# yxtay/transformer-recommenders

Measured on AMD Instinct MI355X. Metric: user-sequences/sec (train step) MovieLens-1M seq200 d128 @1/2/4/8 GPU, higher is better.
Workload: dtype bf16; 1 GPU; MovieLens-1M-shaped: 3883 items, seq_len=200, d_model=128, 4-layer causal BERT (heads=4, ffn=512), InfoNCELoss over in-batch shared negatives, AdamW; per_gpu_batch=512, global_batch=512, seq_len=200, lengths=dense, loss_heads_evaluated=all 7 + LogitsStatistics (reference training_step), parallelism=dp1, launch=eager launches

## Files before the change

### transformer-recommenders_amd/csrc/encoder.hip

```cpp
#include <math.h>
#include <stdlib.h>
#include <new>
#include <string.h>

#include "internal.h"

namespace {

struct LayerParams {
  int64_t wqkv, bqkv, wo, bo, ln1g, ln1b, w1, b1, w2, b2, ln2g, ln2b;
};
struct ParamLayout {
  int64_t pos, type, eg, eb;
  int64_t total;
};

int64_t layer_base(const xfmr_encoder_cfg* c, int i, ParamLayout* pl) {
  const int64_t H = c->hidden, I = c->inter;
  pl->pos = 0;
  pl->type = pl->pos + (int64_t)c->max_pos * H;
  pl->eg = pl->type + 2 * H;
  pl->eb = pl->eg + H;
  const int64_t first = pl->eb + H;
  const int64_t per = 3 * H * H + 3 * H + H * H + H + 2 * H + I * H + I + H * I + H + 2 * H;
// ... 48 lines not shown
  const int64_t i = (int64_t)blockIdx.x * 256 + threadIdx.x;
  if (i < n4) xf_st4<true>(dst, 4 * i, *reinterpret_cast<const float4*>(src + 4 * i));
}

bool mixed_storage(const xfmr_encoder_cfg* c) {
  static const bool force_fp32 = [] {
    const char* e = getenv("XFMR_ACT_FP32");
    return e && *e && *e != '0';
  }();
  return c->precision == XFMR_PREC_BF16 && !force_fp32;
}
int prof(const xfmr_encoder_cfg* c, int kind, int layer, int which, hipStream_t st) {
  if (c->profile_kernel != kind || c->profile_layer != layer || !c->profile_events[which]) return XFMR_OK;
  return hipEventRecord((hipEvent_t)c->profile_events[which], st) == hipSuccess ? XFMR_OK : XFMR_EHIP;
}
bool ln_fused(const xfmr_encoder_cfg* c, int64_t T) {
  static const int64_t min_tokens = [] { const char* e = getenv("XFMR_LN_FUSED_MIN_TOKENS"); return e ? (int64_t)atoll(e) : (int64_t)12288; }();
  return mixed_storage(c) && c->hidden == 128 && T >= min_tokens && !(c->flags & XFMR_ENC_LN_UNFUSED);
}
bool ln_store_x() {
  const char* e = getenv("XFMR_LN_STORE_X");
  return e && *e && *e != '0';
}
bool ffn_fused(const xfmr_encoder_cfg* c, int64_t T) {
  return ln_fused(c, T) && T >= 16384 && (c->inter % 128) == 0 && c->inter <= 1024 && !(c->flags & XFMR_ENC_FFN_UNFUSED);
}

constexpr int64_t kDwSideTokens = 40960;
bool dw_side_shape(const xfmr_encoder_cfg* c, int64_t T) {
  if (!mixed_storage(c) || c->layers > 64) return false;
  return (c->flags & XFMR_ENC_DW_SIDE_ANY) || (c->hidden == 128 && T >= kDwSideTokens);
}

Acts carve(const xfmr_encoder_cfg* c, unsigned char* base, int layer, LayerActs* la, RedBufs* rb = nullptr) {
  const size_t T = (size_t)c->batch * c->seq_len, H = c->hidden, I = c->inter, A = c->heads;
  const size_t es = mixed_storage(c) ? 2 : 4;
  size_t o = 0;
  auto take_bytes = [&](size_t bytes) -> void* {
    void* p = base ? base + o : nullptr;
    o += up256(bytes);
// ... 185 lines not shown
  if (acts_bytes < a.total) return XFMR_EWORKSPACE;
  const int B = cfg->batch, L = cfg->seq_len, H = cfg->hidden, I = cfg->inter, A = cfg->heads;
  const int64_t Tplan = (int64_t)B * L;
  const int32_t* const offs = cfg->seq_offsets;
  const int64_t T = offs ? cfg->packed_rows : Tplan;
  const int prec = cfg->precision;
  const bool mix = mixed_storage(cfg);
  const bool causal = !(cfg->flags & XFMR_ENC_BIDIRECTIONAL);
  hipStream_t st = (hipStream_t)stream;
  const XfSeed sd(cfg->seed, cfg->step_device);
  ParamLayout pl;
  layer_base(cfg, 0, &pl);
  const bool fuse_ln = ln_fused(cfg, Tplan);
  const bool fuse_ffn = ffn_fused(cfg, Tplan);
  const bool rederive = fuse_ln && !ln_store_x();
  float* const x0 = rederive ? nullptr : a.x0;
  if (offs) {
    XF_TRY(xf_embed_ln_fwd_packed_ex(item_idx, table, n_rows, params + pl.pos, params + pl.type, params + pl.eg,
                                     params + pl.eb, x0, mix ? a.x0b : nullptr, a.emb_pre, a.emb_mean, a.emb_rstd, key_mask,
                                     T, cfg->row_pos, H, cfg->ln_eps, cfg->hidden_dropout, sd, SITE_EMB, st));
  } else {
    XF_TRY(xf_embed_ln_fwd_ex(item_idx, table, n_rows, params + pl.pos, params + pl.type, params + pl.eg,
                              params + pl.eb, x0, mix ? a.x0b : nullptr, a.emb_pre, a.emb_mean, a.emb_rstd, key_mask, B,
                              L, H, cfg->ln_eps, cfg->hidden_dropout, sd, SITE_EMB, st));
  }
  if (cfg->embed_event && hipEventRecord((hipEvent_t)cfg->embed_event, st) != hipSuccess) return XFMR_EHIP;
  const float* x = x0;
  XfLnResidual xr{a.emb_pre, a.emb_mean, a.emb_rstd, params + pl.eg, params + pl.eb, cfg->hidden_dropout, SITE_EMB};
  const void* xg = mix ? a.x0b : (const void*)a.x0;
  const uint32_t sA = mix ? XF_S16_A : 0;
// ... 294 lines not shown
```

### transformer-recommenders_amd/csrc/gemm.hip

```cpp
#include <stdio.h>
#include <stdlib.h>

#include <algorithm>
#include <type_traits>

#include "internal.h"

#define XF_PIN_SCALAR(x) asm volatile("" : "+v"(x))
#ifndef XF_LN_DIAG
#define XF_LN_DIAG 0
#endif
#ifndef XF_GEMM_PF
#define XF_GEMM_PF 1
#endif
#ifndef XF_DW_PF
#define XF_DW_PF 1
#endif
#ifdef XF_FFN_STAMP
#define XF_STAMP(i) do { if (stamp_on) st_buf[(i)] = __builtin_readcyclecounter(); } while (0)
#else
#define XF_STAMP(i) do {} while (0)
#endif
#ifndef XF_FFN_ASM_BARRIER
#define XF_FFN_ASM_BARRIER 1
// ... 20 lines not shown

namespace {

enum { EPI_STORE = 0, EPI_GELU = 1, EPI_DROP_RES = 2, EPI_GELU_GRAD = 3, EPI_SPLITK = 4, EPI_DROP_RES_LN = 5,
       EPI_DX_LNBWD = 6, EPI_DROP_RES_LN_RE = 7, EPI_DROP_RES_LN_RED = 8 };
constexpr bool epi_res_ln(int epi) { return epi == EPI_DROP_RES_LN || epi == EPI_DROP_RES_LN_RE || epi == EPI_DROP_RES_LN_RED; }
constexpr int epi_res_mode(int epi) { return epi == EPI_DROP_RES_LN_RE ? 1 : epi == EPI_DROP_RES_LN_RED ? 2 : 0; }

struct GemmArgs {
  const void* A; const void* B; void* C;
  int64_t lda, ldb, ldc;
  int64_t M; int N; int K;
  int k_chunk;
  int nt_n, nt_m, nt_z;
  int nt_full, short_rows;
  const float* bias;
  const float* R;
  const void* P;
  void* C2;
  int aux_grad;
  uint32_t s16;
  float* bias_part;
  XfDropout drop;
  const float* ln_gamma; const float* ln_beta; float ln_eps;
  float* Y; void* Y16; float* ln_mean; float* ln_rstd;
  const float* rp_pre; const float* rp_mean; const float* rp_rstd; const float* rp_gamma; const float* rp_beta;
  XfDropout rp_drop;
  const float* lnb_x; const float* lnb_mean; const float* lnb_rstd;
  void* D16; float* lnb_partials;
  XfDropout drop2;
// ... 201 lines not shown
  return n;
}
static void xf_plan_row_tiles(GemmArgs& g, int BM) {
  g.nt_full = 0; g.short_rows = 0;
  g.nt_m = (int)((g.M + BM - 1) / BM);
  static const bool on = [] { const char* e = getenv("XFMR_ROW_TILES_SHORT"); return e && *e && *e != '0'; }();
  const int64_t cus = xf_num_cus();
  const int64_t per_cu = g.M / (BM * cus), rem = g.M - per_cu * BM * cus;
  if (!on || per_cu < 1 || rem <= 0 || rem > 32 * cus) return;
  const int64_t each = (((rem + cus - 1) / cus) + 15) / 16 * 16;
  g.nt_full = (int)(per_cu * cus);
  g.short_rows = (int)each;
  g.nt_m = g.nt_full + (int)((rem + each - 1) / each);
}

template <int RES>
__device__ __forceinline__ void epi_drop_res_ln_64x128(const f32x16 (&acc)[2], unsigned char* smem, const GemmArgs& g,
                                                       const int64_t m0, const int wid, const int lane) {
  constexpr int LPRL = 16, RPPL = 4, NPL = 4, WM = 32, WN = 64, NI = 2, SCR_LD = WN + 4;
  constexpr int64_t LDC = 128;
  const int wr = wid >> 1, wc = wid & 1;
  float* const scr = reinterpret_cast<float*>(smem) + wid * (16 * SCR_LD);
  float* const red = reinterpret_cast<float*>(smem) + 4 * 16 * SCR_LD;
  const int prow = lane / LPRL, li = lane % LPRL, c0 = li * 4;
  const int n = wc * WN + c0;
  const float4 bias = g.bias ? *reinterpret_cast<const float4*>(g.bias + n) : make_float4(0, 0, 0, 0);
  float4 gp = make_float4(0, 0, 0, 0), bp = gp;
  if constexpr (RES != 0) {
    gp = *reinterpret_cast<const float4*>(g.rp_gamma + n);
    bp = *reinterpret_cast<const float4*>(g.rp_beta + n);
  }
  float4 vv[2][NPL];
#pragma unroll
  for (int hf = 0; hf < 2; ++hf) {
    const int64_t mb = m0 + wr * WM + 16 * hf;
    float4 aux[NPL];
    float amu[NPL], ars[NPL];
#pragma unroll
    for (int ps = 0; ps < NPL; ++ps) {
      aux[ps] = make_float4(0, 0, 0, 0);
      amu[ps] = ars[ps] = 0.f;
      const int64_t m = mb + prow + RPPL * ps;
      if constexpr (RES == 0) {
        if (m < g.M) aux[ps] = *reinterpret_cast<const float4*>(g.R + m * LDC + n);
      } else if (m < g.M) {
        aux[ps] = *reinterpret_cast<const float4*>(g.rp_pre + m * LDC + n);
        amu[ps] = g.rp_mean[m];
        ars[ps] = g.rp_rstd[m];
      }
    }
#pragma unroll
    for (int j = 0; j < NI; ++j)
#pragma unroll
      for (int r = 0; r < 8; ++r)
        scr[(xf_acc_row(8 * hf + r, lane) - 16 * hf) * SCR_LD + j * 32 + (lane & 31)] = acc[j][8 * hf + r];
    __builtin_amdgcn_s_waitcnt(0xc07f);
    __builtin_amdgcn_wave_barrier();
#pragma unroll
    for (int ps = 0; ps < NPL; ++ps) {
      const int row = prow + RPPL * ps;
      const int64_t m = mb + row;
      float4 v = *reinterpret_cast<const float4*>(scr + row * SCR_LD + c0);
      v.x += bias.x; v.y += bias.y; v.z += bias.z; v.w += bias.w;
      if (g.drop.on) {
        xf_drop4(g.drop, (uint32_t)m, (uint32_t)(n), v);
      }
      float4 res = aux[ps];
      if constexpr (RES != 0) {
        XF_PIN_SCALAR(amu[ps]);
        XF_PIN_SCALAR(ars[ps]);
        res = xf_ln_out_drop4<RES == 2>(res, amu[ps], ars[ps], gp, bp, g.rp_drop, (uint32_t)m, (uint32_t)(n));
      }
      v.x += res.x; v.y += res.y; v.z += res.z; v.w += res.w;
      if (m >= g.M) v = make_float4(0, 0, 0, 0);
      else *reinterpret_cast<float4*>(reinterpret_cast<float*>(g.C) + m * LDC + n) = v;
      vv[hf][ps] = v;
    }
    __builtin_amdgcn_s_waitcnt(0xc07f);
    __builtin_amdgcn_wave_barrier();
  }
  XF_EPI_BARRIER();
  auto row_reduce = [&](float x) { return xf_row16_sum(x); };
  float mean[2][NPL];
#pragma unroll
  for (int hf = 0; hf < 2; ++hf)
#pragma unroll
    for (int ps = 0; ps < NPL; ++ps) {
      const float4 v = vv[hf][ps];
      const float s = row_reduce((v.x + v.y) + (v.z + v.w));
      if (li == 0) red[(wr * 2 + wc) * 32 + 16 * hf + prow + RPPL * ps] = s;
    }
  XF_EPI_BARRIER();
#pragma unroll
  for (int hf = 0; hf < 2; ++hf)
#pragma unroll
    for (int ps = 0; ps < NPL; ++ps) {
      const int rr = 16 * hf + prow + RPPL * ps;
      mean[hf][ps] = (red[(wr * 2) * 32 + rr] + red[(wr * 2 + 1) * 32 + rr]) * (1.f / 128.f);
    }
  XF_EPI_BARRIER();
#pragma unroll
  for (int hf = 0; hf < 2; ++hf)
#pragma unroll
    for (int ps = 0; ps < NPL; ++ps) {
      float4& v = vv[hf][ps];
      const float mu = mean[hf][ps];
      v.x -= mu; v.y -= mu; v.z -= mu; v.w -= mu;
      const float s = row_reduce((v.x * v.x + v.y * v.y) + (v.z * v.z + v.w * v.w));
      if (li == 0) red[(wr * 2 + wc) * 32 + 16 * hf + prow + RPPL * ps] = s;
    }
  XF_EPI_BARRIER();
  const float4 gm = *reinterpret_cast<const float4*>(g.ln_gamma + n);
  const float4 bt = *reinterpret_cast<const float4*>(g.ln_beta + n);
#pragma unroll
  for (int hf = 0; hf < 2; ++hf)
#pragma unroll
    for (int ps = 0; ps < NPL; ++ps) {
      const int rr = 16 * hf + prow + RPPL * ps;
      const int64_t m = m0 + wr * WM + rr;
      const float var = (red[(wr * 2) * 32 + rr] + red[(wr * 2 + 1) * 32 + rr]) * (1.f / 128.f);
      const float rs = rsqrtf(var + g.ln_eps);
      if (m >= g.M) continue;
      const float4 o = xf_ln_affine4(vv[hf][ps], rs, gm, bt);
      if (g.Y) *reinterpret_cast<float4*>(g.Y + m * LDC + n) = o;
      if (g.Y16) xf_st4<true>(g.Y16, m * LDC + n, o);
      if (wc == 0 && li == 0) {
        g.ln_mean[m] = mean[hf][ps];
        g.ln_rstd[m] = rs;
      }
    }
}

__device__ __forceinline__ void epi_dx_lnbwd_64x128(const f32x16 (&acc)[2], unsigned char* smem, const GemmArgs& g,
// ... 94 lines not shown
#pragma unroll
    for (int o = LPRL; o < 64; o <<= 1) {
      v.x += __shfl_xor(v.x, o, 64); v.y += __shfl_xor(v.y, o, 64);
      v.z += __shfl_xor(v.z, o, 64); v.w += __shfl_xor(v.w, o, 64);
    }
  };
  fold(dgam); fold(dbet); fold(dbias);
  if (prow == 0) {
    *reinterpret_cast<float4*>(&colred[(wr * 3 + 0) * 128 + n]) = dgam;
    *reinterpret_cast<float4*>(&colred[(wr * 3 + 1) * 128 + n]) = dbet;
    *reinterpret_cast<float4*>(&colred[(wr * 3 + 2) * 128 + n]) = dbias;
  }
  XF_EPI_BARRIER();
  for (int o = threadIdx.x; o < 3 * 128; o += 256)
    g.lnb_partials[(int64_t)tile_m * 3 * 128 + o] = colred[o] + colred[3 * 128 + o];
}

template <class P, int BM, int BN, int BK, bool TA, bool TB, int EPI, uint32_t S>
__device__ __forceinline__ void gemm_body(const GemmArgs& g_in, const int bid) {
  GemmArgs g = g_in;
  if (EPI != EPI_SPLITK) XF_CHAIN_PRIO();
  g.drop = xf_drop_resolve(g.drop); g.drop2 = xf_drop_resolve(g.drop2);
  if constexpr (EPI == EPI_DROP_RES_LN_RED) g.rp_drop = xf_drop_resolve(g.rp_drop);
  using elem = typename P::elem;
  using TileA = OperandTile<P, BM, BK, TA>;
  using TileB = OperandTile<P, BN, BK, TB>;
  using FA = Frag<P, TA>;
  using FB = Frag<P, TB>;
  constexpr bool a16 = S & XF_S16_A, b16 = S & XF_S16_B, c16 = S & XF_S16_C, p16 = S & XF_S16_P;
  static_assert(S == 0 || sizeof(elem) == 2, "bf16 storage needs the bf16 policy");
// ... 2 lines not shown
  constexpr size_t SCR_BYTES = (size_t)4 * 16 * SCR_LD * sizeof(float);
  constexpr size_t RED_BYTES = epi_res_ln(EPI) ? (size_t)4 * 32 * sizeof(float)
                               : EPI == EPI_DX_LNBWD  ? (size_t)(2 * 2 * 2 * 16 * 2 + 2 * 3 * 128) * sizeof(float)
                                                      : 0;
  constexpr size_t EPI_BYTES = SCR_BYTES + RED_BYTES;
  __shared__ __attribute__((aligned(16))) unsigned char smem[OPER_BYTES > EPI_BYTES ? OPER_BYTES : EPI_BYTES];
  elem* const sA = reinterpret_cast<elem*>(smem);
  elem* const sB = sA + TileA::IMG_ELEMS;

  const int lane = threadIdx.x & 63, wid = threadIdx.x >> 6;
  const int wr = wid >> 1, wc = wid & 1;
  constexpr int WM = BM / 2, WN = BN / 2, MI = WM / 32, NI = WN / 32;
  const TileIdx tix = tile_of(g.nt_n, g.nt_m, g.nt_z, bid);
  if (!tix.valid) return;
  const int64_t m0 = (epi_res_ln(EPI) || EPI == EPI_DX_LNBWD) ? xf_tile_rows(g, tix.m, BM) : (int64_t)tix.m * BM;
  const int n0 = tix.n * BN;
  int kbeg = 0, kend = g.K;
  if (g.k_chunk > 0) {
    kbeg = tix.z * g.k_chunk;
    kend = min(g.K, kbeg + g.k_chunk);
  }

  f32x16 acc[MI][NI];
#pragma unroll
  for (int i = 0; i < MI; ++i)
#pragma unroll
    for (int j = 0; j < NI; ++j)
#pragma unroll
      for (int r = 0; r < 16; ++r) acc[i][j][r] = 0.f;

// ... 231 lines not shown
    xf_static_for<NW>([&](auto ic) {
      constexpr int i = decltype(ic)::value;
      const int p = tid + i * 256, row = p / PC, ch = p % PC;
      reg[i] = *reinterpret_cast<const bf16x8*>(W2 + (int64_t)row * I + c * CH + ch * 8);
    });
  }
  __device__ __forceinline__ void commit_w2(__bf16* sW, int tid) const {
    xf_static_for<NW>([&](auto ic) {
      constexpr int i = decltype(ic)::value;
      const int p = tid + i * 256, row = p / PC, ch = p % PC;
      *reinterpret_cast<bf16x8*>(sW + row * LDC + ch * 8) = reg[i];
    });
  }
};

template <int CH, bool RE = false>
__global__ __launch_bounds__(256, CH == 128 ? XF_FFN_MIN_WAVES : 3) void ffn_fwd_fused_kernel(const FfnFwdArgs f_in) {
  FfnFwdArgs f = f_in;
  XF_CHAIN_PRIO();
  f.e.drop = xf_drop_resolve(f.e.drop);
  constexpr int H = 128, LDH = H + 8, LDC = CH + 8, BM = 64;
  constexpr int NJ = CH / 64;
  constexpr int W_ELEMS = CH * LDH > H * LDC ? CH * LDH : H * LDC;
  __shared__ __attribute__((aligned(16))) __bf16 sG[BM * LDC];
  __shared__ __attribute__((aligned(16))) __bf16 sW[W_ELEMS];
  __shared__ float sB1[1024];
  static_assert(W_ELEMS >= BM * LDH, "the x tile is staged through sW");
  static_assert(W_ELEMS * 2 >= 4 * 16 * 68 * 4 + 128 * 4, "the LayerNorm epilogue's scratch aliases sW");
  using FR = Frag<PrecBF16, false>;
  const int lane = threadIdx.x & 63, wid = threadIdx.x >> 6, tid = threadIdx.x;
  const int wr = wid >> 1, wc = wid & 1;
  const TileIdx tix = tile_of(1, f.e.nt_m, 1);
  if (!tix.valid) return;
  const int64_t m0 = xf_tile_rows(f.e, tix.m, BM);
  const int64_t M = f.e.M;
  const int I = f.I, nchunk = I / CH;
#ifdef XF_FFN_STAMP
  const bool stamp_on = f.stamps && threadIdx.x == 0;
  unsigned long long* st_buf = f.stamps + (int64_t)blockIdx.x * 64;
#endif
  XF_STAMP(0);

  WeightChunk<CH> wa, wb;
  constexpr int PC = CH / 8;

  {
    uint4 xr[4];
#pragma unroll
    for (int i = 0; i < 4; ++i) {
      const int p = tid + i * 256, row = p >> 4, ch = p & 15;
      xr[i] = make_uint4(0u, 0u, 0u, 0u);
      if (m0 + row < M) xr[i] = *reinterpret_cast<const uint4*>(f.X + (m0 + row) * H + ch * 8);
    }
    wa.load_w1(f.W1, 0, tid);
    wb.load_w2(f.W2, I, 0, tid);
    for (int i = tid; i < I; i += 256) sB1[i] = f.b1[i];
#pragma unroll
    for (int i = 0; i < 4; ++i) {
      const int p = tid + i * 256, row = p >> 4, ch = p & 15;
      *reinterpret_cast<uint4*>(sW + row * LDH + ch * 8) = xr[i];
    }
  }
  __syncthreads();
  bf16x8 xa[H / 16];
#pragma unroll
  for (int ks = 0; ks < H / 16; ++ks) xa[ks] = FR::get(sW, LDH, wr * 32, ks * 16);
  XF_STAMP(1);

  f32x16 accy[2];
#pragma unroll
  for (int j = 0; j < 2; ++j)
#pragma unroll
    for (int r = 0; r < 16; ++r) accy[j][r] = 0.f;

  for (int c = 0; c < nchunk; ++c) {
    XF_LOOP_BARRIER();
    if (c < 2) XF_STAMP(2 + 6 * c);
    wa.commit_w1(sW, tid);
    XF_LOOP_BARRIER();
    if (c < 2) XF_STAMP(3 + 6 * c);
    if (c + 1 < nchunk) wa.load_w1(f.W1, c + 1, tid);
    f32x16 accu[NJ];
#pragma unroll
    for (int j = 0; j < NJ; ++j)
#pragma unroll
      for (int r = 0; r < 16; ++r) accu[j][r] = 0.f;
    {
      bf16x8 fb[2][NJ];
#pragma unroll
      for (int j = 0; j < NJ; ++j) fb[0][j] = FR::get(sW, LDH, wc * (CH / 2) + j * 32, 0);
#pragma unroll
      for (int ks = 0; ks < H / 16; ++ks) {
        if (ks + 1 < H / 16) {
#pragma unroll
          for (int j = 0; j < NJ; ++j) fb[(ks + 1) & 1][j] = FR::get(sW, LDH, wc * (CH / 2) + j * 32, (ks + 1) * 16);
        }
#pragma unroll
        for (int j = 0; j < NJ; ++j) accu[j] = xf_mma(xa[ks], fb[ks & 1][j], accu[j]);
      }
    }
#pragma unroll
    for (int j = 0; j < NJ; ++j) {
      const int col = wc * (CH / 2) + j * 32 + (lane & 31);
      const float b = sB1[c * CH + col];
#pragma unroll
      for (int r = 0; r < 16; ++r) sG[(wr * 32 + xf_acc_row(r, lane)) * LDC + col] = (__bf16)(accu[j][r] + b);
    }
    if (c < 2) XF_STAMP(4 + 6 * c);
    XF_LOOP_BARRIER();
    if (c < 2) XF_STAMP(5 + 6 * c);
#pragma unroll
    for (int i = 0; i < BM * PC / 256; ++i) {
      const int p = tid + i * 256, row = p / PC, ch = p % PC;
      float4* cell = reinterpret_cast<float4*>(sG + row * LDC + ch * 8);
      const float4 u8 = *cell;
      const float4 g8 = xf_gelu_bf16x8(u8);
      if (m0 + row < M) {
        if (f.U) *reinterpret_cast<float4*>(f.U + (m0 + row) * I + c * CH + ch * 8) = u8;
        if (f.G) *reinterpret_cast<float4*>(f.G + (m0 + row) * I + c * CH + ch * 8) = g8;
      }
      *cell = g8;
    }
    wb.commit_w2(sW, tid);
    if (c < 2) XF_STAMP(6 + 6 * c);
    XF_LOOP_BARRIER();
    if (c < 2) XF_STAMP(7 + 6 * c);
    if (c + 1 < nchunk) wb.load_w2(f.W2, I, c + 1, tid);
#pragma unroll
    for (int ks = 0; ks < CH / 16; ++ks) {
      const bf16x8 fa = FR::get(sG, LDC, wr * 32, ks * 16);
      bf16x8 fb[2];
#pragma unroll
      for (int j = 0; j < 2; ++j) fb[j] = FR::get(sW, LDC, wc * 64 + j * 32, ks * 16);
#pragma unroll
      for (int j = 0; j < 2; ++j) accy[j] = xf_mma(fa, fb[j], accy[j]);
    }
  }
  XF_STAMP(14);
  __syncthreads();
  XF_STAMP(15);
  epi_drop_res_ln_64x128<RE ? 1 : 0>(accy, reinterpret_cast<unsigned char*>(sW), f.e, m0, wid, lane);
  XF_STAMP(16);
}

struct FfnBwdArgs {
  const __bf16* DY;
  const __bf16* W2;
  const __bf16* U;
  const __bf16* W1;
  __bf16* DI;
  int I;
  GemmArgs e;
};

__global__ __launch_bounds__(256, 3) void ffn_bwd_dx_fused_kernel(const FfnBwdArgs f_in) {
  FfnBwdArgs f = f_in;
  XF_CHAIN_PRIO();
// ... 278 lines not shown
    static const TileOverride dw = [] {
      TileOverride o{0, 0, 0};
      if (const char* e = getenv("XFMR_DW_TILE")) sscanf(e, "%d,%d", &o.bm, &o.bn);
      return o;
    }();
    if (dw.bm) { bm = dw.bm; bn = dw.bn; }
  }
  const TileOverride ov = tile_override();
  if (ov.bm && !epi_res_ln(EPI) && EPI != EPI_DX_LNBWD) { bm = ov.bm; bn = ov.bn; }
  dim3 block(256);
  static const int pad_lds = [] { const char* e = getenv("XFMR_GEMM_PAD_LDS"); return e ? atoi(e) : 0; }();
  GemmArgs ga = g;
  ga.nt_n = (int)((g.N + bn - 1) / bn);
  ga.nt_m = (int)((g.M + bm - 1) / bm);
  if (epi_res_ln(EPI) || EPI == EPI_DX_LNBWD) xf_plan_row_tiles(ga, bm);
  ga.nt_z = splits;
  const int64_t groups = splits > 1 ? (splits + 7) / 8 : (ga.nt_m + 7) / 8;
  const int64_t per = splits > 1 ? (int64_t)ga.nt_n * ga.nt_m : ga.nt_n;
  if (groups * per * 8 > 0x7fffffffll) return XFMR_EUNSUPPORTED;
  dim3 grid((unsigned)(groups * per * 8));
  if (bm == 64 && bn == 128) hipLaunchKernelGGL((gemm_kernel<P, 64, 128, BK, TA, TB, EPI, S>), grid, block, pad_lds, st, ga);
  else if (bm == 128 && bn == 64) hipLaunchKernelGGL((gemm_kernel<P, 128, 64, BK, TA, TB, EPI, S>), grid, block, pad_lds, st, ga);
  else if (bm == 64) hipLaunchKernelGGL((gemm_kernel<P, 64, 64, BK, TA, TB, EPI, S>), grid, block, pad_lds, st, ga);
  else hipLaunchKernelGGL((gemm_kernel<P, 128, 128, BK, TA, TB, EPI, S>), grid, block, pad_lds, st, ga);
  XF_LAUNCH_CHECK();
  return XFMR_OK;
}

template <class P, bool TA, bool TB, int EPI, uint32_t S>
int launch_gemm(const GemmArgs& g, int splits, hipStream_t st) {
// ... 90 lines not shown
      (b2 && !xf_aligned16(b2)) || !xf_aligned16(gamma) || !xf_aligned16(beta))
    return XFMR_EALIGN;
  FfnFwdArgs f{};
  f.X = (const __bf16*)x16; f.W1 = (const __bf16*)w1_16; f.b1 = b1; f.W2 = (const __bf16*)w2_16; f.U = (__bf16*)u16; f.G = (__bf16*)g16;
  f.I = I;
#ifdef XF_FFN_STAMP
  if (const char* e = getenv("XFMR_FFN_STAMPS")) f.stamps = (unsigned long long*)strtoull(e, nullptr, 0);
#endif
  GemmArgs& g = f.e;
  g.C = pre; g.ldc = H; g.M = M; g.N = H; g.K = I; g.bias = b2;
  if (const int rc = set_ln_residual(g, residual, res, seed)) return rc;
  g.drop = xf_make_dropout(dropout_p, seed, site);
  g.ln_gamma = gamma; g.ln_beta = beta; g.ln_eps = eps; g.Y = y; g.Y16 = y16; g.ln_mean = mean; g.ln_rstd = rstd;
  g.nt_n = 1; g.nt_z = 1;
  xf_plan_row_tiles(g, 64);
  const int64_t groups = (g.nt_m + 7) / 8;
  if (groups * 8 > 0x7fffffffll) return XFMR_EUNSUPPORTED;
  const char* ce = getenv("XFMR_FFN_CHUNK");
  const int chunk = ce ? atoi(ce) : 64;
  const dim3 grid((unsigned)(groups * 8));
  if (chunk == 64 && res) hipLaunchKernelGGL((ffn_fwd_fused_kernel<64, true>), grid, dim3(256), 0, st, f);
  else if (chunk == 64) hipLaunchKernelGGL((ffn_fwd_fused_kernel<64, false>), grid, dim3(256), 0, st, f);
  else if (res) hipLaunchKernelGGL((ffn_fwd_fused_kernel<128, true>), grid, dim3(256), 0, st, f);
  else hipLaunchKernelGGL((ffn_fwd_fused_kernel<128, false>), grid, dim3(256), 0, st, f);
  XF_LAUNCH_CHECK();
  return XFMR_OK;
}

}


extern "C" {

int xf_dw_split_plan(int64_t M, int32_t N, int32_t K, int* k_chunk) { return dw_split_plan(M, N, K, k_chunk); }

int xf_rowsum(float* dst, const float* src, int64_t rows, int64_t cols, hipStream_t st) {
  return launch_rowsum(dst, src, rows, cols, rows, st);
}

int xf_ln_row_tiles(int64_t M) {
  GemmArgs g{};
  g.M = M;
  xf_plan_row_tiles(g, 64);
  return g.nt_m;
}

int xf_linear_fwd_ex(const void* x, const float* w, const float* bias, void* y, int64_t M, int32_t N, int32_t K,
                     int32_t epilogue, const float* residual, void* aux_out, float dropout_p, XfSeed seed,
                     uint32_t site, int32_t precision, uint32_t s16, hipStream_t st) {
  if (!x || !w || !y || M <= 0 || N <= 0 || K <= 0) return XFMR_EINVAL;
  if ((K & 3) || (N & 3)) return XFMR_EUNSUPPORTED;
  if (!xf_aligned16(x) || !xf_aligned16(w) || !xf_aligned16(y)) return XFMR_EALIGN;
// ... 302 lines not shown
```

### transformer-recommenders_amd/csrc/internal.h

```cpp
#pragma once
#include "common.h"

enum : uint32_t {
  XF_S16_A = 1u,
  XF_S16_B = 2u,
  XF_S16_C = 4u,
  XF_S16_P = 8u,
  XF_AUX_GELU_GRAD = 0x100u,
};

extern "C" {
int xf_linear_fwd_ex(const void* x, const float* w, const float* bias, void* y, int64_t M, int32_t N, int32_t K,
                     int32_t epilogue, const float* residual, void* aux_out, float dropout_p, XfSeed seed,
                     uint32_t site, int32_t precision, uint32_t s16, hipStream_t st);
int xf_ffn_fwd_fused_ex(const void* x16, const void* w1_16, const float* b1, const void* w2_16, const float* b2,
                        void* u16, void* g16, float* pre, int64_t M, int32_t H, int32_t I, const float* residual, float dropout_p,
                        XfSeed seed, uint32_t site, const float* gamma, const float* beta, float eps, float* y,
                        void* y16, float* mean, float* rstd, hipStream_t st);
struct XfLnResidual {
  const float* pre; const float* mean; const float* rstd; const float* gamma; const float* beta;
  float dropout_p; uint32_t site;
};
int xf_ffn_fwd_fused_re(const void* x16, const void* w1_16, const float* b1, const void* w2_16, const float* b2,
                        void* u16, void* g16, float* pre, int64_t M, int32_t H, int32_t I, const XfLnResidual* res,
// ... 27 lines not shown
int xf_attn_fwd_ex(const void* qkv, const uint8_t* key_mask, void* ctx, float* lse, int32_t B, int32_t L, int32_t A,
                   int32_t H, float dropout_p, XfSeed seed, uint32_t site, int32_t precision, bool s16,
                   bool causal, hipStream_t st, const int32_t* seq_offsets = nullptr,
                   bool stream_keys = false);
int xf_attn_bwd_ex(const void* qkv, const uint8_t* key_mask, const void* ctx, const float* lse, const void* d_ctx,
                   void* d_qkv, int32_t B, int32_t L, int32_t A, int32_t H, float dropout_p, XfSeed seed,
                   uint32_t site, int32_t precision, bool s16, bool causal, hipStream_t st,
                   const int32_t* seq_offsets = nullptr, bool stream_keys = false);
int xf_loss_finalize(const double* blockpart, int nblocks, int rows_per_block, const int* counts, int mode,
                     int64_t n_rows, int64_t positions, float* losses, float* stats, double* tot, hipStream_t st);
int xf_linear_ln_fwd_ex(const void* x, const float* w, const float* bias, float* pre, int64_t M, int32_t N, int32_t K,
                        const float* residual, float dropout_p, XfSeed seed, uint32_t site, const float* gamma,
                        const float* beta, float eps, float* y, void* y16, float* mean, float* rstd, int32_t precision,
                        uint32_t s16, hipStream_t st);
int xf_ln_row_tiles(int64_t M);
int xf_linear_bwd_dx_lnbwd_ex(const void* dy, const float* w, int64_t M, int32_t N, int32_t K,
                              const float* residual_grad, const float* ln_x, const float* ln_mean, const float* ln_rstd,
                              const float* ln_gamma, float dropout_p, XfSeed seed, uint32_t site, float* dx,
                              void* d_lin16, float* partials, int* blocks_out, int32_t precision, uint32_t s16,
                              hipStream_t st, float out_dropout_p = 0.f, uint32_t out_site = 0);
int xf_layernorm_fwd_ex(const float* x, const float* gamma, const float* beta, float* y, void* y16, float* mean,
                        float* rstd, int64_t rows, int32_t H, float eps, hipStream_t stream);
int xf_embed_ln_fwd_ex(const int64_t* item_idx, const float* table, int64_t n_rows, const float* pos_emb,
                       const float* type_emb, const float* gamma, const float* beta, float* out, void* out16,
                       float* pre, float* mean, float* rstd, uint8_t* key_mask, int32_t B, int32_t L, int32_t H,
                       float eps, float dropout_p, XfSeed seed, uint32_t site, hipStream_t stream);
int xf_embed_ln_fwd_packed_ex(const int64_t* item_idx, const float* table, int64_t n_rows, const float* pos_emb,
                              const float* type_emb, const float* gamma, const float* beta, float* out, void* out16,
                              float* pre, float* mean, float* rstd, uint8_t* key_mask, int64_t rows, const int32_t* row_pos,
                              int32_t H, float eps, float dropout_p, XfSeed seed, uint32_t site, hipStream_t stream);
// ... 8 lines not shown
```

Before: 166,400 sequences/s.

## Split last-wave row tiles into 32-row tiles for fused LN GEMM and FFN

Adds tail-tile planning so that when the 64-row tile count leaves a partial final wave across CUs, the leftover rows are covered by 32-row tiles. The LN-fused GEMM gets an inline 32-row path, and the fused FFN forward gets a separate 32-row tail kernel launched after the main grid. The aim is to cut wave-quantization imbalance, where a few tiles run alone in the last wave. The cost is an extra launch, occupancy queries, and 32-row tiles that use the MMA units less efficiently. An env switch is also added to force fusion at small token counts.

```diff
diff --git a/transformer-recommenders_amd/csrc/encoder.hip b/transformer-recommenders_amd/csrc/encoder.hip
--- a/transformer-recommenders_amd/csrc/encoder.hip
+++ b/transformer-recommenders_amd/csrc/encoder.hip
@@ -86,16 +86,20 @@
   if (c->profile_kernel != kind || c->profile_layer != layer || !c->profile_events[which]) return XFMR_OK;
   return hipEventRecord((hipEvent_t)c->profile_events[which], st) == hipSuccess ? XFMR_OK : XFMR_EHIP;
 }
+bool fuse_any_tokens() {
+  const char* e = getenv("XFMR_FUSE_ANY_TOKENS");
+  return e && *e && *e != '0';
+}
 bool ln_fused(const xfmr_encoder_cfg* c, int64_t T) {
   static const int64_t min_tokens = [] { const char* e = getenv("XFMR_LN_FUSED_MIN_TOKENS"); return e ? (int64_t)atoll(e) : (int64_t)12288; }();
-  return mixed_storage(c) && c->hidden == 128 && T >= min_tokens && !(c->flags & XFMR_ENC_LN_UNFUSED);
+  return mixed_storage(c) && c->hidden == 128 && (T >= min_tokens || fuse_any_tokens()) && !(c->flags & XFMR_ENC_LN_UNFUSED);
 }
 bool ln_store_x() {
   const char* e = getenv("XFMR_LN_STORE_X");
   return e && *e && *e != '0';
 }
 bool ffn_fused(const xfmr_encoder_cfg* c, int64_t T) {
-  return ln_fused(c, T) && T >= 16384 && (c->inter % 128) == 0 && c->inter <= 1024 && !(c->flags & XFMR_ENC_FFN_UNFUSED);
+  return ln_fused(c, T) && (T >= 16384 || fuse_any_tokens()) && (c->inter % 128) == 0 && c->inter <= 1024 && !(c->flags & XFMR_ENC_FFN_UNFUSED);
 }
 
 constexpr int64_t kDwSideTokens = 40960;
@@ -311,6 +315,7 @@
   const bool fuse_ln = ln_fused(cfg, Tplan);
   const bool fuse_ffn = ffn_fused(cfg, Tplan);
   const bool rederive = fuse_ln && !ln_store_x();
+  if (fuse_ln) xf_tail_tiles_refresh();
   float* const x0 = rederive ? nullptr : a.x0;
   if (offs) {
     XF_TRY(xf_embed_ln_fwd_packed_ex(item_idx, table, n_rows, params + pl.pos, params + pl.type, params + pl.eg,
diff --git a/transformer-recommenders_amd/csrc/gemm.hip b/transformer-recommenders_amd/csrc/gemm.hip
--- a/transformer-recommenders_amd/csrc/gemm.hip
+++ b/transformer-recommenders_amd/csrc/gemm.hip
@@ -58,6 +58,7 @@
   int k_chunk;
   int nt_n, nt_m, nt_z;
   int nt_full, short_rows;
+  int tail32;
   const float* bias;
   const float* R;
   const void* P;
@@ -289,14 +290,47 @@
   g.nt_m = g.nt_full + (int)((rem + each - 1) / each);
 }
 
-template <int RES>
-__device__ __forceinline__ void epi_drop_res_ln_64x128(const f32x16 (&acc)[2], unsigned char* smem, const GemmArgs& g,
+struct TailTiles { bool on; int slots; };
+static TailTiles xf_read_tail_tiles() {
+  const char* e = getenv("XFMR_TAIL_TILES");
+  const char* s = getenv("XFMR_TAIL_SLOTS");
+  return TailTiles{!(e && *e == '0'), s ? atoi(s) : 0};
+}
+static TailTiles& xf_tail_tiles() {
+  static TailTiles t = xf_read_tail_tiles();
+  return t;
+}
+template <class K>
+static int xf_wg_per_cu(K kernel) {
+  int n = 0;
+  if (hipOccupancyMaxActiveBlocksPerMultiprocessor(&n, kernel, 256, 0) != hipSuccess || n < 1) n = 1;
+  return n;
+}
+static void xf_plan_tail_tiles(GemmArgs& g, int wg_per_cu) {
+  g.tail32 = 0;
+  const TailTiles t = xf_tail_tiles();
+  if (!t.on || g.nt_full > 0) return;
+  const int64_t slots = t.slots > 0 ? t.slots : (int64_t)xf_num_cus() * wg_per_cu;
+  if (g.nt_m < slots) return;
+  const int tail = (int)(g.nt_m % slots);
+  if (tail == 0) return;
+  g.nt_full = g.nt_m - tail;
+  g.short_rows = 32;
+  g.tail32 = 1;
+  g.nt_m = g.nt_full + (int)((g.M - (int64_t)g.nt_full * 64 + 31) / 32);
+}
+
+template <int RES, bool T32 = false>
+__device__ __forceinline__ void epi_drop_res_ln_64x128(const f32x16* acc, unsigned char* smem, const GemmArgs& g,
                                                        const int64_t m0, const int wid, const int lane) {
   constexpr int LPRL = 16, RPPL = 4, NPL = 4, WM = 32, WN = 64, NI = 2, SCR_LD = WN + 4;
+  constexpr int NHF = T32 ? 1 : 2, TLD = 128 + 4;
   constexpr int64_t LDC = 128;
-  const int wr = wid >> 1, wc = wid & 1;
+  const int wr = T32 ? 0 : wid >> 1, wc = wid & 1;
+  const int h0 = T32 ? wid >> 1 : 0;
   float* const scr = reinterpret_cast<float*>(smem) + wid * (16 * SCR_LD);
   float* const red = reinterpret_cast<float*>(smem) + 4 * 16 * SCR_LD;
+  static_assert(32 * TLD <= 4 * 16 * SCR_LD, "the 32-row image must end before the exchange records");
   const int prow = lane / LPRL, li = lane % LPRL, c0 = li * 4;
   const int n = wc * WN + c0;
   const float4 bias = g.bias ? *reinterpret_cast<const float4*>(g.bias + n) : make_float4(0, 0, 0, 0);
@@ -305,10 +339,10 @@
     gp = *reinterpret_cast<const float4*>(g.rp_gamma + n);
     bp = *reinterpret_cast<const float4*>(g.rp_beta + n);
   }
-  float4 vv[2][NPL];
-#pragma unroll
-  for (int hf = 0; hf < 2; ++hf) {
-    const int64_t mb = m0 + wr * WM + 16 * hf;
+  float4 vv[NHF][NPL];
+#pragma unroll
+  for (int hf = 0; hf < NHF; ++hf) {
+    const int64_t mb = m0 + wr * WM + 16 * (h0 + hf);
     float4 aux[NPL];
     float amu[NPL], ars[NPL];
 #pragma unroll
@@ -324,18 +358,26 @@
         ars[ps] = g.rp_rstd[m];
       }
     }
-#pragma unroll
-    for (int j = 0; j < NI; ++j)
-#pragma unroll
-      for (int r = 0; r < 8; ++r)
-        scr[(xf_acc_row(8 * hf + r, lane) - 16 * hf) * SCR_LD + j * 32 + (lane & 31)] = acc[j][8 * hf + r];
-    __builtin_amdgcn_s_waitcnt(0xc07f);
-    __builtin_amdgcn_wave_barrier();
+    if constexpr (!T32) {
+#pragma unroll
+      for (int j = 0; j < NI; ++j)
+#pragma unroll
+        for (int r = 0; r < 8; ++r)
+          scr[(xf_acc_row(8 * hf + r, lane) - 16 * hf) * SCR_LD + j * 32 + (lane & 31)] = acc[j][8 * hf + r];
+      __builtin_amdgcn_s_waitcnt(0xc07f);
+      __builtin_amdgcn_wave_barrier();
+    } else {
+#pragma unroll
+      for (int r = 0; r < 16; ++r)
+        reinterpret_cast<float*>(smem)[xf_acc_row(r, lane) * TLD + wid * 32 + (lane & 31)] = acc[0][r];
+      XF_EPI_BARRIER();
+    }
 #pragma unroll
     for (int ps = 0; ps < NPL; ++ps) {
       const int row = prow + RPPL * ps;
       const int64_t m = mb + row;
-      float4 v = *reinterpret_cast<const float4*>(scr + row * SCR_LD + c0);
+      float4 v = T32 ? *reinterpret_cast<const float4*>(reinterpret_cast<const float*>(smem) + (16 * h0 + row) * TLD + n)
+                     : *reinterpret_cast<const float4*>(scr + row * SCR_LD + c0);
       v.x += bias.x; v.y += bias.y; v.z += bias.z; v.w += bias.w;
       if (g.drop.on) {
         xf_drop4(g.drop, (uint32_t)m, (uint32_t)(n), v);
@@ -356,42 +398,42 @@
   }
   XF_EPI_BARRIER();
   auto row_reduce = [&](float x) { return xf_row16_sum(x); };
-  float mean[2][NPL];
-#pragma unroll
-  for (int hf = 0; hf < 2; ++hf)
+  float mean[NHF][NPL];
+#pragma unroll
+  for (int hf = 0; hf < NHF; ++hf)
 #pragma unroll
     for (int ps = 0; ps < NPL; ++ps) {
       const float4 v = vv[hf][ps];
       const float s = row_reduce((v.x + v.y) + (v.z + v.w));
-      if (li == 0) red[(wr * 2 + wc) * 32 + 16 * hf + prow + RPPL * ps] = s;
+      if (li == 0) red[(wr * 2 + wc) * 32 + 16 * (h0 + hf) + prow + RPPL * ps] = s;
     }
   XF_EPI_BARRIER();
 #pragma unroll
-  for (int hf = 0; hf < 2; ++hf)
+  for (int hf = 0; hf < NHF; ++hf)
 #pragma unroll
     for (int ps = 0; ps < NPL; ++ps) {
-      const int rr = 16 * hf + prow + RPPL * ps;
+      const int rr = 16 * (h0 + hf) + prow + RPPL * ps;
       mean[hf][ps] = (red[(wr * 2) * 32 + rr] + red[(wr * 2 + 1) * 32 + rr]) * (1.f / 128.f);
     }
   XF_EPI_BARRIER();
 #pragma unroll
-  for (int hf = 0; hf < 2; ++hf)
+  for (int hf = 0; hf < NHF; ++hf)
 #pragma unroll
     for (int ps = 0; ps < NPL; ++ps) {
       float4& v = vv[hf][ps];
       const float mu = mean[hf][ps];
       v.x -= mu; v.y -= mu; v.z -= mu; v.w -= mu;
       const float s = row_reduce((v.x * v.x + v.y * v.y) + (v.z * v.z + v.w * v.w));
-      if (li == 0) red[(wr * 2 + wc) * 32 + 16 * hf + prow + RPPL * ps] = s;
+      if (li == 0) red[(wr * 2 + wc) * 32 + 16 * (h0 + hf) + prow + RPPL * ps] = s;
     }
   XF_EPI_BARRIER();
   const float4 gm = *reinterpret_cast<const float4*>(g.ln_gamma + n);
   const float4 bt = *reinterpret_cast<const float4*>(g.ln_beta + n);
 #pragma unroll
-  for (int hf = 0; hf < 2; ++hf)
+  for (int hf = 0; hf < NHF; ++hf)
 #pragma unroll
     for (int ps = 0; ps < NPL; ++ps) {
-      const int rr = 16 * hf + prow + RPPL * ps;
+      const int rr = 16 * (h0 + hf) + prow + RPPL * ps;
       const int64_t m = m0 + wr * WM + rr;
       const float var = (red[(wr * 2) * 32 + rr] + red[(wr * 2 + 1) * 32 + rr]) * (1.f / 128.f);
       const float rs = rsqrtf(var + g.ln_eps);
@@ -516,6 +558,46 @@
   XF_EPI_BARRIER();
   for (int o = threadIdx.x; o < 3 * 128; o += 256)
     g.lnb_partials[(int64_t)tile_m * 3 * 128 + o] = colred[o] + colred[3 * 128 + o];
+}
+
+template <class P, int BM, int BN, int BK, bool TA, bool TB, int EPI, uint32_t S>
+constexpr bool gemm_has_tail32() {
+  return epi_res_ln(EPI) && sizeof(typename P::elem) == 2 && BM == 64 && BN == 128 && BK == 64 && !TA && !TB &&
+         S == (XF_S16_A | XF_S16_B);
+}
+template <class P, int BK, int EPI>
+__device__ __forceinline__ void gemm_tail32_ln(const GemmArgs& g, unsigned char* smem, const int64_t m0) {
+  using elem = typename P::elem;
+  using TileA = OperandTile<P, 32, BK, false>;
+  using TileB = OperandTile<P, 128, BK, false>;
+  using FR = Frag<P, false>;
+  elem* const sA = reinterpret_cast<elem*>(smem);
+  elem* const sB = sA + TileA::IMG_ELEMS;
+  const int lane = threadIdx.x & 63, wid = threadIdx.x >> 6;
+  f32x16 acc;
+#pragma unroll
+  for (int r = 0; r < 16; ++r) acc[r] = 0.f;
+  TileA ta;
+  TileB tb;
+  const int nk = (g.K + BK - 1) / BK;
+  ta.template load<true>(g.A, g.lda, m0, g.M, 0, g.K);
+  tb.template load<true>(g.B, g.ldb, 0, g.N, 0, g.K);
+#pragma unroll 1
+  for (int kt = 0; kt < nk; ++kt) {
+    __syncthreads();
+    ta.template commit<true>(sA);
+    tb.template commit<true>(sB);
+    __syncthreads();
+    if (kt + 1 < nk) {
+      ta.template load<true>(g.A, g.lda, m0, g.M, (kt + 1) * BK, g.K);
+      tb.template load<true>(g.B, g.ldb, 0, g.N, (kt + 1) * BK, g.K);
+    }
+#pragma unroll
+    for (int k0 = 0; k0 < BK; k0 += FR::KS)
+      acc = xf_mma(FR::get(sA, TileA::LD, 0, k0), FR::get(sB, TileB::LD, wid * 32, k0), acc);
+  }
+  __syncthreads();
+  epi_drop_res_ln_64x128<epi_res_mode(EPI), true>(&acc, smem, g, m0, wid, lane);
 }
 
 template <class P, int BM, int BN, int BK, bool TA, bool TB, int EPI, uint32_t S>
@@ -548,6 +630,12 @@
   const TileIdx tix = tile_of(g.nt_n, g.nt_m, g.nt_z, bid);
   if (!tix.valid) return;
   const int64_t m0 = (epi_res_ln(EPI) || EPI == EPI_DX_LNBWD) ? xf_tile_rows(g, tix.m, BM) : (int64_t)tix.m * BM;
+  if constexpr (gemm_has_tail32<P, BM, BN, BK, TA, TB, EPI, S>()) {
+    if (g.tail32 && tix.m >= g.nt_full) {
+      gemm_tail32_ln<P, BK, EPI>(g, smem, m0);
+      return;
+    }
+  }
   const int n0 = tix.n * BN;
   int kbeg = 0, kend = g.K;
   if (g.k_chunk > 0) {
@@ -809,25 +897,23 @@
   }
 };
 
-template <int CH, bool RE = false>
-__global__ __launch_bounds__(256, CH == 128 ? XF_FFN_MIN_WAVES : 3) void ffn_fwd_fused_kernel(const FfnFwdArgs f_in) {
-  FfnFwdArgs f = f_in;
-  XF_CHAIN_PRIO();
-  f.e.drop = xf_drop_resolve(f.e.drop);
-  constexpr int H = 128, LDH = H + 8, LDC = CH + 8, BM = 64;
-  constexpr int NJ = CH / 64;
-  constexpr int W_ELEMS = CH * LDH > H * LDC ? CH * LDH : H * LDC;
-  __shared__ __attribute__((aligned(16))) __bf16 sG[BM * LDC];
-  __shared__ __attribute__((aligned(16))) __bf16 sW[W_ELEMS];
-  __shared__ float sB1[1024];
-  static_assert(W_ELEMS >= BM * LDH, "the x tile is staged through sW");
-  static_assert(W_ELEMS * 2 >= 4 * 16 * 68 * 4 + 128 * 4, "the LayerNorm epilogue's scratch aliases sW");
+constexpr int ffn_w_elems(int CH) { return CH * (128 + 8) > 128 * (CH + 8) ? CH * (128 + 8) : 128 * (CH + 8); }
+constexpr int ffn_g_elems(int BM, int CH) { return BM * (CH + 8); }
+
+template <int CH, int BM, bool RE>
+__device__ __forceinline__ void ffn_fwd_tile(const FfnFwdArgs& f, __bf16* const sG, __bf16* const sW, float* const sB1,
+                                             const int64_t m0) {
+  constexpr bool T32 = BM == 32;
+  static_assert(BM == 64 || (T32 && CH == 128), "a 32-row tile walks I in 128-column chunks");
+  constexpr int H = 128, LDH = H + 8, LDC = CH + 8;
+  constexpr int NJ = T32 ? 1 : CH / 64;
+  constexpr int NY = T32 ? 1 : 2;
+  constexpr int XP = BM * 16 / 256;
   using FR = Frag<PrecBF16, false>;
   const int lane = threadIdx.x & 63, wid = threadIdx.x >> 6, tid = threadIdx.x;
-  const int wr = wid >> 1, wc = wid & 1;
-  const TileIdx tix = tile_of(1, f.e.nt_m, 1);
-  if (!tix.valid) return;
-  const int64_t m0 = xf_tile_rows(f.e, tix.m, BM);
+  const int wr = T32 ? 0 : wid >> 1;
+  const int cu0 = T32 ? wid * 32 : (wid & 1) * (CH / 2);
+  const int cy0 = T32 ? wid * 32 : (wid & 1) * 64;
   const int64_t M = f.e.M;
   const int I = f.I, nchunk = I / CH;
 #ifdef XF_FFN_STAMP
@@ -840,9 +926,9 @@
   constexpr int PC = CH / 8;
 
   {
-    uint4 xr[4];
-#pragma unroll
-    for (int i = 0; i < 4; ++i) {
+    uint4 xr[XP];
+#pragma unroll
+    for (int i = 0; i < XP; ++i) {
       const int p = tid + i * 256, row = p >> 4, ch = p & 15;
       xr[i] = make_uint4(0u, 0u, 0u, 0u);
       if (m0 + row < M) xr[i] = *reinterpret_cast<const uint4*>(f.X + (m0 + row) * H + ch * 8);
@@ -851,7 +937,7 @@
     wb.load_w2(f.W2, I, 0, tid);
     for (int i = tid; i < I; i += 256) sB1[i] = f.b1[i];
 #pragma unroll
-    for (int i = 0; i < 4; ++i) {
+    for (int i = 0; i < XP; ++i) {
       const int p = tid + i * 256, row = p >> 4, ch = p & 15;
       *reinterpret_cast<uint4*>(sW + row * LDH + ch * 8) = xr[i];
     }
@@ -862,9 +948,9 @@
   for (int ks = 0; ks < H / 16; ++ks) xa[ks] = FR::get(sW, LDH, wr * 32, ks * 16);
   XF_STAMP(1);
 
-  f32x16 accy[2];
-#pragma unroll
-  for (int j = 0; j < 2; ++j)
+  f32x16 accy[NY];
+#pragma unroll
+  for (int j = 0; j < NY; ++j)
 #pragma unroll
     for (int r = 0; r < 16; ++r) accy[j][r] = 0.f;
 
@@ -883,12 +969,12 @@
     {
       bf16x8 fb[2][NJ];
 #pragma unroll
-      for (int j = 0; j < NJ; ++j) fb[0][j] = FR::get(sW, LDH, wc * (CH / 2) + j * 32, 0);
+      for (int j = 0; j < NJ; ++j) fb[0][j] = FR::get(sW, LDH, cu0 + j * 32, 0);
 #pragma unroll
       for (int ks = 0; ks < H / 16; ++ks) {
         if (ks + 1 < H / 16) {
 #pragma unroll
-          for (int j = 0; j < NJ; ++j) fb[(ks + 1) & 1][j] = FR::get(sW, LDH, wc * (CH / 2) + j * 32, (ks + 1) * 16);
+          for (int j = 0; j < NJ; ++j) fb[(ks + 1) & 1][j] = FR::get(sW, LDH, cu0 + j * 32, (ks + 1) * 16);
         }
 #pragma unroll
         for (int j = 0; j < NJ; ++j) accu[j] = xf_mma(xa[ks], fb[ks & 1][j], accu[j]);
@@ -896,7 +982,7 @@
     }
 #pragma unroll
     for (int j = 0; j < NJ; ++j) {
-      const int col = wc * (CH / 2) + j * 32 + (lane & 31);
+      const int col = cu0 + j * 32 + (lane & 31);
       const float b = sB1[c * CH + col];
 #pragma unroll
       for (int r = 0; r < 16; ++r) sG[(wr * 32 + xf_acc_row(r, lane)) * LDC + col] = (__bf16)(accu[j][r] + b);
@@ -924,18 +1010,49 @@
 #pragma unroll
     for (int ks = 0; ks < CH / 16; ++ks) {
       const bf16x8 fa = FR::get(sG, LDC, wr * 32, ks * 16);
-      bf16x8 fb[2];
-#pragma unroll
-      for (int j = 0; j < 2; ++j) fb[j] = FR::get(sW, LDC, wc * 64 + j * 32, ks * 16);
-#pragma unroll
-      for (int j = 0; j < 2; ++j) accy[j] = xf_mma(fa, fb[j], accy[j]);
+      bf16x8 fb[NY];
+#pragma unroll
+      for (int j = 0; j < NY; ++j) fb[j] = FR::get(sW, LDC, cy0 + j * 32, ks * 16);
+#pragma unroll
+      for (int j = 0; j < NY; ++j) accy[j] = xf_mma(fa, fb[j], accy[j]);
     }
   }
   XF_STAMP(14);
   __syncthreads();
   XF_STAMP(15);
-  epi_drop_res_ln_64x128<RE ? 1 : 0>(accy, reinterpret_cast<unsigned char*>(sW), f.e, m0, wid, lane);
+  epi_drop_res_ln_64x128<RE ? 1 : 0, T32>(accy, reinterpret_cast<unsigned char*>(sW), f.e, m0, wid, lane);
   XF_STAMP(16);
+}
+
+template <int CH, bool RE = false>
+__global__ __launch_bounds__(256, CH == 128 ? XF_FFN_MIN_WAVES : 3) void ffn_fwd_fused_kernel(const FfnFwdArgs f_in) {
+  FfnFwdArgs f = f_in;
+  XF_CHAIN_PRIO();
+  f.e.drop = xf_drop_resolve(f.e.drop);
+  constexpr int W_ELEMS = ffn_w_elems(CH);
+  __shared__ __attribute__((aligned(16))) __bf16 sG[ffn_g_elems(64, CH)];
+  __shared__ __attribute__((aligned(16))) __bf16 sW[W_ELEMS];
+  __shared__ float sB1[1024];
+  static_assert(W_ELEMS >= 64 * (128 + 8), "the x tile is staged through sW");
+  static_assert(W_ELEMS * 2 >= 4 * 16 * 68 * 4 + 128 * 4, "the LayerNorm epilogue's scratch aliases sW");
+  const TileIdx tix = tile_of(1, f.e.nt_m, 1);
+  if (!tix.valid) return;
+  const int64_t m0 = xf_tile_rows(f.e, tix.m, 64);
+  ffn_fwd_tile<CH, 64, RE>(f, sG, sW, sB1, m0);
+}
+template <bool RE>
+__global__ __launch_bounds__(256, 2) void ffn_fwd_tail32_kernel(const FfnFwdArgs f_in) {
+  FfnFwdArgs f = f_in;
+  XF_CHAIN_PRIO();
+  f.e.drop = xf_drop_resolve(f.e.drop);
+  __shared__ __attribute__((aligned(16))) __bf16 sG[ffn_g_elems(32, 128)];
+  __shared__ __attribute__((aligned(16))) __bf16 sW[ffn_w_elems(128)];
+  __shared__ float sB1[1024];
+  static_assert(ffn_w_elems(128) * 2 >= 4 * 16 * 68 * 4 + 128 * 4, "the LayerNorm epilogue's scratch aliases sW");
+  const int m = f.e.nt_full + (int)blockIdx.x;
+  if (m >= f.e.nt_m) return;
+  const int64_t m0 = xf_tile_rows(f.e, m, 64);
+  ffn_fwd_tile<128, 32, RE>(f, sG, sW, sB1, m0);
 }
 
 struct FfnBwdArgs {
@@ -1244,6 +1361,10 @@
   ga.nt_n = (int)((g.N + bn - 1) / bn);
   ga.nt_m = (int)((g.M + bm - 1) / bm);
   if (epi_res_ln(EPI) || EPI == EPI_DX_LNBWD) xf_plan_row_tiles(ga, bm);
+  if constexpr (gemm_has_tail32<P, 64, 128, BK, TA, TB, EPI, S>()) {
+    static const int wg_per_cu = xf_wg_per_cu(gemm_kernel<P, 64, 128, BK, TA, TB, EPI, S>);
+    if (bm == 64 && bn == 128) xf_plan_tail_tiles(ga, wg_per_cu);
+  }
   ga.nt_z = splits;
   const int64_t groups = splits > 1 ? (splits + 7) / 8 : (ga.nt_m + 7) / 8;
   const int64_t per = splits > 1 ? (int64_t)ga.nt_n * ga.nt_m : ga.nt_n;
@@ -1364,16 +1485,28 @@
   g.ln_gamma = gamma; g.ln_beta = beta; g.ln_eps = eps; g.Y = y; g.Y16 = y16; g.ln_mean = mean; g.ln_rstd = rstd;
   g.nt_n = 1; g.nt_z = 1;
   xf_plan_row_tiles(g, 64);
+  const char* ce = getenv("XFMR_FFN_CHUNK");
+  const int chunk = ce ? atoi(ce) : 64;
+  if (chunk == 64) {
+    static const int wg_per_cu[2] = {xf_wg_per_cu(ffn_fwd_fused_kernel<64, false>), xf_wg_per_cu(ffn_fwd_fused_kernel<64, true>)};
+    xf_plan_tail_tiles(g, wg_per_cu[res ? 1 : 0]);
+  }
+  FfnFwdArgs ft = f;
+  if (g.tail32) { g.nt_m = g.nt_full; g.nt_full = 0; g.short_rows = 0; g.tail32 = 0; }
   const int64_t groups = (g.nt_m + 7) / 8;
   if (groups * 8 > 0x7fffffffll) return XFMR_EUNSUPPORTED;
-  const char* ce = getenv("XFMR_FFN_CHUNK");
-  const int chunk = ce ? atoi(ce) : 64;
   const dim3 grid((unsigned)(groups * 8));
   if (chunk == 64 && res) hipLaunchKernelGGL((ffn_fwd_fused_kernel<64, true>), grid, dim3(256), 0, st, f);
   else if (chunk == 64) hipLaunchKernelGGL((ffn_fwd_fused_kernel<64, false>), grid, dim3(256), 0, st, f);
   else if (res) hipLaunchKernelGGL((ffn_fwd_fused_kernel<128, true>), grid, dim3(256), 0, st, f);
   else hipLaunchKernelGGL((ffn_fwd_fused_kernel<128, false>), grid, dim3(256), 0, st, f);
   XF_LAUNCH_CHECK();
+  if (ft.e.tail32) {
+    const dim3 tgrid((unsigned)(ft.e.nt_m - ft.e.nt_full));
+    if (res) hipLaunchKernelGGL((ffn_fwd_tail32_kernel<true>), tgrid, dim3(256), 0, st, ft);
+    else hipLaunchKernelGGL((ffn_fwd_tail32_kernel<false>), tgrid, dim3(256), 0, st, ft);
+    XF_LAUNCH_CHECK();
+  }
   return XFMR_OK;
 }
 
@@ -1386,6 +1519,16 @@
 
 int xf_rowsum(float* dst, const float* src, int64_t rows, int64_t cols, hipStream_t st) {
   return launch_rowsum(dst, src, rows, cols, rows, st);
+}
+
+void xf_tail_tiles_refresh() { xf_tail_tiles() = xf_read_tail_tiles(); }
+int xf_tail_tiles_plan(int64_t M, int wg_per_cu, int* full_tiles) {
+  GemmArgs g{};
+  g.M = M;
+  xf_plan_row_tiles(g, 64);
+  xf_plan_tail_tiles(g, wg_per_cu);
+  if (full_tiles) *full_tiles = g.tail32 ? g.nt_full : g.nt_m;
+  return g.tail32 ? g.nt_m - g.nt_full : 0;
 }
 
 int xf_ln_row_tiles(int64_t M) {
diff --git a/transformer-recommenders_amd/csrc/internal.h b/transformer-recommenders_amd/csrc/internal.h
--- a/transformer-recommenders_amd/csrc/internal.h
+++ b/transformer-recommenders_amd/csrc/internal.h
@@ -65,6 +65,8 @@
                         const float* beta, float eps, float* y, void* y16, float* mean, float* rstd, int32_t precision,
                         uint32_t s16, hipStream_t st);
 int xf_ln_row_tiles(int64_t M);
+void xf_tail_tiles_refresh();
+int xf_tail_tiles_plan(int64_t M, int wg_per_cu, int* full_tiles);
 int xf_linear_bwd_dx_lnbwd_ex(const void* dy, const float* w, int64_t M, int32_t N, int32_t K,
                               const float* residual_grad, const float* ln_x, const float* ln_mean, const float* ln_rstd,
                               const float* ln_gamma, float dropout_p, XfSeed seed, uint32_t site, float* dx,
```

Measured after the change: 164,700 sequences/s. -1.0%, worse.
